# zhoujun-7/VPHO

Measured on AMD Instinct MI355X. Metric: eval images/sec (bs=64, sample_num=100, steps=50); MPJPE delta vs ref, higher is better.
Workload: dtype f32; 1 GPU; vpho_net.forward(mode=predict), README eval config (BASELINE.json configs[1]); per_gpu_batch=64, sample_num=100, sampling_steps=50, topk_hand=30, topk_obj=10, crop=256x256, pipeline_depth=3, parallelism=dp1, score_mfma=f32, conv_mfma=f32, winograd_3x3=True

## Files before the change

### vpho_amd/csrc/conv_igemm.hip

```cpp
#include "common.h"
#include "../../include/vpho_hip.h"
#include <cstdlib>
#include <algorithm>

VPHO_STAMP_DECL(conv)

namespace {

#ifndef CONV_ABLATE
#define CONV_ABLATE 0
#endif
constexpr int BK = 32;
constexpr int LDS_LD = BK + 4;
constexpr int GLDS_PRE_MAX = 512;

struct Geo {
    vpho_conv_desc d;
    int M, K, tiles_m, tiles_n, ntiles;
    int w_ld;
    long long x_zs, w_zs, y_zs;
    long long b_zs, r_zs, x2_zs, pre_zs, ru_zs;
    int y_linear, r_linear, vec_epilogue;
    int uni;
    int dbg;
// ... 540 lines not shown
#pragma unroll
                for (int i = 0; i < TM; ++i)
#pragma unroll
                    for (int j = 0; j < TN; ++j)
                        acc[i][j] = __builtin_amdgcn_mfma_f32_32x32x2f32(a[i][q], b[j][q], acc[i][j], 0, 0, 0);
        }
    };
    VPHO_STAMP_AT(2);
    VPHO_PRIO_MAIN();
    for (int kt = 0; kt + 1 < nk; ++kt) {
        if ((kt > 0 || (g.dbg & 16)) && !(CONV_ABLATE & 64)) { if (UNI) fill_uni((kt & 1) ^ 1, kt + 1); else fill((kt & 1) ^ 1); }
        compute(kt);
        if (!(CONV_ABLATE & 128)) VPHO_SYNC_LDS_DMA();
    }
    if (res_early) { if (d.res_up) load_res_up(); else load_res(); __builtin_amdgcn_sched_barrier(0); }
    compute(nk - 1);
    VPHO_SYNC_LDS_DMA();
    VPHO_PRIO_REST();
    VPHO_STAMP_AT(3);
    if ((CONV_ABLATE & 256) && acc[0][0][0] != 1.2345e-30f) return;

    if (g.vec_epilogue) {
        constexpr int C_LD = BN;
        float* Cs = smem;
        static_assert(BM * C_LD <= 2 * TILE, "epilogue tile does not fit the staging LDS");
#pragma unroll
        for (int j = 0; j < TN; ++j)
#pragma unroll
            for (int i = 0; i < TM; ++i)
#pragma unroll
                for (int e = 0; e < 16; ++e) {
                    const int r = wm * (BM / WM) + i * 32 + (e & 3) + 8 * (e >> 2) + 4 * lh;
                    Cs[r * C_LD + wn * (BN / WN) + j * 32 + li] = acc[i][j][e];
                }
        __syncthreads();
        if (!res_early) { if (d.res_up) load_res_up(); else load_res(); }
        static_assert(NT % V_PER_ROW == 0 && NT >= 2 * BN, "stats layout");
        f32x4 st0 = {0.f, 0.f, 0.f, 0.f}, st1 = {0.f, 0.f, 0.f, 0.f}, piv = st0;
        float cnt = 0.f;
        f32x4 bn_m = st0, bn_i = st0, bn_g = st0, bn_b = st0;
        if (d.bn_x) {
            const int c = n0 + 4 * (tid % V_PER_ROW);
            if (c < d.Cout) {
                bn_m = *reinterpret_cast<const f32x4*>(d.bn_mean + c); bn_i = *reinterpret_cast<const f32x4*>(d.bn_invstd + c);
                if (!d.gate) { bn_g = *reinterpret_cast<const f32x4*>(d.bn_gamma + c); bn_b = *reinterpret_cast<const f32x4*>(d.bn_beta + c); }
            }
        }
#pragma unroll
        for (int it = 0; it < ITERS; ++it) {
            long long yoff, ro;
            if (!item(it, yoff, ro)) continue;
            const int idx = tid + it * NT;
            const int r = idx / V_PER_ROW, c4 = idx - r * V_PER_ROW;
            const f32x4 v = *reinterpret_cast<const f32x4*>(Cs + r * C_LD + 4 * c4);
            f32x4 bv = {0.f, 0.f, 0.f, 0.f};
            if (d.bias) bv = *reinterpret_cast<const f32x4*>(d.bias + n0 + 4 * c4);
            f32x4 o;
#pragma unroll
            for (int k = 0; k < 4; ++k) { const float t = v[k] + bv[k] + rv[it][k]; o[k] = t > 0.f ? t : t * d.out_slope; }
            if (d.gate) {
                const f32x4 gt = *reinterpret_cast<const f32x4*>(d.gate + yoff);
#pragma unroll
                for (int k = 0; k < 4; ++k) o[k] = gt[k] > 0.f ? o[k] : o[k] * d.gate_slope;
            }
            if (d.bn_x) {
                const f32x4 xv = *reinterpret_cast<const f32x4*>(d.bn_x + yoff);
#pragma unroll
                for (int k = 0; k < 4; ++k) {
                    const float xh = (xv[k] - bn_m[k]) * bn_i[k];
                    if (!d.gate) {
                        const float t = xh * bn_g[k] + bn_b[k];
                        o[k] = t > 0.f ? o[k] : o[k] * d.gate_slope;
                    }
                    st0[k] += o[k]; st1[k] += o[k] * xh;
                }
            } else if (d.stats) {
                if (it == 0) {
#pragma unroll
                    for (int k = 0; k < 4; ++k) piv[k] = __shfl(o[k], lane & (V_PER_ROW - 1));
                }
                cnt += 1.f;
#pragma unroll
                for (int k = 0; k < 4; ++k) { const float dv = o[k] - piv[k]; st0[k] += dv; st1[k] += dv * dv; }
            }
            *reinterpret_cast<f32x4*>(d.y + yoff) = o;
        }
        if (d.stats) {
            static_assert(V_PER_ROW == 16 || V_PER_ROW == 32, "lane layout of the epilogue items");
            constexpr int NWAVES = NT / 64;
            static_assert(4 * NWAVES * BN <= BM * C_LD, "stats staging");
#pragma unroll
            for (int k = 0; k < 4; ++k) {
                if (V_PER_ROW == 16) { st0[k] = sum_lane_bit_4(st0[k]); st1[k] = sum_lane_bit_4(st1[k]); }
                st0[k] = sum_lane_bit_5(st0[k]); st1[k] = sum_lane_bit_5(st1[k]);
            }
            if (!d.bn_x) {
                if (V_PER_ROW == 16) cnt = sum_lane_bit_4(cnt);
                cnt = sum_lane_bit_5(cnt);
            }
            __syncthreads();
            float* R = smem;
            if (lane < V_PER_ROW) {
                *reinterpret_cast<f32x4*>(R + (wave * 4 + 0) * BN + 4 * lane) = st0;
                *reinterpret_cast<f32x4*>(R + (wave * 4 + 1) * BN + 4 * lane) = st1;
                *reinterpret_cast<f32x4*>(R + (wave * 4 + 2) * BN + 4 * lane) = piv;
                *reinterpret_cast<f32x4*>(R + (wave * 4 + 3) * BN + 4 * lane) = f32x4{cnt, cnt, cnt, cnt};
            }
            __syncthreads();
            if (d.bn_x) {
                if (tid < 2 * BN) {
                    const int pl = tid / BN, c = tid - pl * BN;
                    float t = R[pl * BN + c];
#pragma unroll
                    for (int k = 1; k < NWAVES; ++k) t += R[(k * 4 + pl) * BN + c];
                    if (n0 + c < d.Cout) d.stats[((long long)tile_m * BN_STAT_PLANES + pl) * d.Cout + n0 + c] = t;
                }
            } else if (tid < BN) {
                const int c = tid;
                ShiftSums t{R[2 * BN + c], R[c], R[BN + c], R[3 * BN + c]};
#pragma unroll
                for (int k = 1; k < NWAVES; ++k) t = shift_sums_add(t, ShiftSums{R[(k * 4 + 2) * BN + c], R[(k * 4) * BN + c], R[(k * 4 + 1) * BN + c], R[(k * 4 + 3) * BN + c]});
                if (n0 + c < d.Cout) store_bn_row(d.stats + (long long)tile_m * BN_STAT_PLANES * d.Cout + n0 + c, d.Cout, t);
            }
        }
        VPHO_STAMP_AT(4);
        VPHO_STAMP_WRITE(conv, blockIdx.x);
        return;
    }
    const int row_base = m0 + wm * (BM / WM) + 4 * lh, col_base = n0 + wn * (BN / WN) + li;
#pragma unroll
    for (int j = 0; j < TN; ++j) {
        const int col = col_base + j * 32;
        if (col >= d.Cout) continue;
        const float bv = d.bias ? d.bias[col] : 0.f;
#pragma unroll
        for (int i = 0; i < TM; ++i) {
#pragma unroll
            for (int e = 0; e < 16; ++e) {
                const int row = row_base + i * 32 + (e & 3) + 8 * (e >> 2);
                if (row >= M_live) continue;
                long long yoff, ro;
                offsets(row, yoff, ro);
                float v = acc[i][j][e] + bv;
                if (d.res) v += d.res[ro + col];
                v = v > 0.f ? v : v * d.out_slope;
                if (d.gate) v = d.gate[yoff + col] > 0.f ? v : v * d.gate_slope;
                d.y[yoff + col] = v;
            }
        }
    }
}

#define VPHO_WAIT_VM(n) asm volatile("s_waitcnt vmcnt(%0)" :: "n"(n) : "memory")
template <int BM, int BN, int WM, int WN, bool STATS>
__device__ __forceinline__ void conv_pers_body(const Geo& g) {
    constexpr int NT = 64 * WM * WN, NW = WM * WN;
    constexpr int TM = BM / (32 * WM), TN = BN / (32 * WN);
    constexpr int ROWS = NT / 8;
    constexpr int A_LD = BM / ROWS, B_LD = BN / ROWS, NF = A_LD + B_LD;
    static_assert(TM >= 1 && TN >= 1 && A_LD >= 1 && B_LD >= 1 && ROWS % 16 == 0 && BN / WN <= 64, "tile/wave layout");
    constexpr int TILE = (BM + BN) * BK;
    constexpr int EPI = 8 * 32;
    constexpr int NIT = TM * 4 * TN;
    __shared__ __attribute__((aligned(1024))) float smem[2 * TILE + NW * EPI + 2 * BN];
    VPHO_STAMP_INIT();

    vpho_conv_desc d = g.d;
    advance_group(d, g, blockIdx.y);
    const int tid = threadIdx.x, lane = tid & 63, wave = __builtin_amdgcn_readfirstlane(tid >> 6);
    const int li = lane & 31, lh = lane >> 5;
    const int wm = wave / WN, wn = wave % WN;
    const int lrow = wave * 8 + (lane >> 3);
    const int kq = (lane & 7) ^ ((lrow >> 1) & 7);
    const int ohw = d.OH * d.OW;
    const __amdgpu_buffer_rsrc_t xu = __builtin_amdgcn_make_buffer_rsrc(const_cast<float*>(d.x), 0, 0xFFFFFFF0u, 0x00020000);
    const __amdgpu_buffer_rsrc_t wr = __builtin_amdgcn_make_buffer_rsrc(const_cast<float*>(d.w), 0, 0xFFFFFFF0u, 0x00020000);
    const __amdgpu_buffer_rsrc_t x2r = __builtin_amdgcn_make_buffer_rsrc(const_cast<float*>(d.x2 ? d.x2 : d.x), 0, 0xFFFFFFF0u, 0x00020000);
    const __amdgpu_buffer_rsrc_t yr = __builtin_amdgcn_make_buffer_rsrc(d.y, 0, 0xFFFFFFF0u, 0x00020000);
    const __amdgpu_buffer_rsrc_t rr = __builtin_amdgcn_make_buffer_rsrc(const_cast<float*>(d.res ? d.res : d.y), 0, 0xFFFFFFF0u, 0x00020000);
    const __amdgpu_buffer_rsrc_t br = __builtin_amdgcn_make_buffer_rsrc(const_cast<float*>(d.bias ? d.bias : d.w), 0, 0xFFFFFFF0u, 0x00020000);
    typedef __attribute__((address_space(3))) void* lds_ptr;

    const int xcd = blockIdx.x & 7, nslot = gridDim.x >> 3, per_xcd = (g.ntiles + 7) >> 3;
    int lt = blockIdx.x >> 3;
    auto tile_at = [&](int t, int& m0, int& n0) -> bool {
        const int lb = xcd * per_xcd + t;
        if (t >= per_xcd || lb >= g.ntiles) return false;
        const int tile_m = lb / g.tiles_n, tile_n = lb - tile_m * g.tiles_n;
        m0 = tile_m * BM; n0 = tile_n * BN;
        return true;
    };
    int m0, n0;
    if (!tile_at(lt, m0, n0)) return;

    int u_voff[A_LD], u_boff[B_LD], u_voff2[A_LD], bias_off;
    auto setup = [&](int m0_, int n0_) {
#pragma unroll
        for (int j = 0; j < A_LD; ++j) {
            const int m = m0_ + lrow + ROWS * j;
            u_voff[j] = -1; u_voff2[j] = -1;
            if (m < g.M) {
                const int n = m / ohw, rem = m - n * ohw;
                const int oy = rem / d.OW, ox = rem - oy * d.OW;
                u_voff[j] = (int)((((long long)(n * d.H + oy * d.stride) * d.W + ox * d.stride) * d.x_ld) * 4 + 16 * kq);
                if (d.x2) u_voff2[j] = (int)((((long long)(n * d.H2 + oy * d.stride2) * d.W2 + ox * d.stride2) * d.x2_ld) * 4 + 16 * kq);
            }
        }
#pragma unroll
        for (int j = 0; j < B_LD; ++j) {
            const int n = n0_ + lrow + ROWS * j;
            u_boff[j] = n < d.Cout ? (int)(((long long)n * g.w_ld + 4 * kq) * 4) : -1;
        }
        const int bc = n0_ + wn * (BN / WN) + lane;
        bias_off = (d.bias && lane < BN / WN && bc < d.Cout) ? bc * 4 : -1;
    };
    auto fill = [&](int buf, int kt, int tp) {
        float* As = smem + buf * TILE + wave * 8 * BK;
        float* Bs = smem + buf * TILE + BM * BK + wave * 8 * BK;
        if (d.x2 && kt * BK >= d.Cin) {
            const int c2 = (kt * BK - d.Cin) * 4;
#pragma unroll
            for (int j = 0; j < A_LD; ++j) {
                const int vo = u_voff2[j];
                __builtin_amdgcn_raw_ptr_buffer_load_lds(x2r, (lds_ptr)(As + ROWS * j * BK), 16, vo, c2, 0, 0);
            }
        } else {
            const int c1 = kt * BK * 4;
#pragma unroll
            for (int j = 0; j < A_LD; ++j) {
                const int vo = u_voff[j];
                __builtin_amdgcn_raw_ptr_buffer_load_lds(xu, (lds_ptr)(As + ROWS * j * BK), 16, vo, c1, 0, 0);
            }
        }
        const int koff = kt * BK * 4;
#pragma unroll
        for (int j = 0; j < B_LD; ++j) {
            const int bo = u_boff[j];
            __builtin_amdgcn_raw_ptr_buffer_load_lds(wr, (lds_ptr)(Bs + ROWS * j * BK), 16, bo, koff, 0, 0);
        }
        if (kt == 0) {
            const int bo = bias_off;
            __builtin_amdgcn_raw_ptr_buffer_load_lds(br, (lds_ptr)(smem + 2 * TILE + NW * EPI + tp * BN + wn * (BN / WN)), 4, bo, 0, 0, 0);
        }
    };

    const int nk = (g.K + BK - 1) / BK;
    const int sw = (li >> 1) & 7;
    f32x16 acc[TM][TN];
    auto compute = [&](int kt) {
        const int buf = kt & 1;
        const float* As = smem + buf * TILE + (wm * (BM / WM) + li) * BK;
        const float* Bs = smem + buf * TILE + BM * BK + (wn * (BN / WN) + li) * BK;
#pragma unroll
        for (int kk = 0; kk < BK / 8; ++kk) {
            const int ch = ((2 * kk + lh) ^ sw) * 4;
            f32x4 a[TM], b[TN];
#pragma unroll
            for (int i = 0; i < TM; ++i) a[i] = *reinterpret_cast<const f32x4*>(As + i * 32 * BK + ch);
#pragma unroll
            for (int j = 0; j < TN; ++j) b[j] = *reinterpret_cast<const f32x4*>(Bs + j * 32 * BK + ch);
#pragma unroll
            for (int q = 0; q < 4; ++q)
#pragma unroll
                for (int i = 0; i < TM; ++i)
#pragma unroll
                    for (int j = 0; j < TN; ++j)
                        acc[i][j] = __builtin_amdgcn_mfma_f32_32x32x2f32(a[i][q], b[j][q], acc[i][j], 0, 0, 0);
        }
    };

    float* Cw = smem + 2 * TILE + wave * EPI;
    const int er = lane >> 3, ec = (lane & 7) * 4;
    auto item_off = [&](int m0_, int n0_, int i, int gq, int j, int& yo, int& ro) {
        const int row = m0_ + wm * (BM / WM) + i * 32 + 8 * gq + er, col = n0_ + wn * (BN / WN) + j * 32 + ec;
        yo = ro = -1;
        if (row < g.M && col < d.Cout) {
            long long y_, r_;
            if (g.y_linear && g.r_linear) { y_ = (long long)row * d.y_sx; r_ = (long long)row * d.r_sx; }
            else {
                const int n = row / ohw, rem = row - n * ohw;
                const int oy = rem / d.OW, ox = rem - oy * d.OW;
                y_ = n * d.y_sn + oy * d.y_sy + ox * d.y_sx; r_ = n * d.r_sn + oy * d.r_sy + ox * d.r_sx;
            }
            yo = (int)((y_ + col) * 4);
            if (d.res) ro = (int)((r_ + col) * 4);
        }
    };

    constexpr bool stats_on = STATS;
    static_assert(4 * (BN / WN) <= EPI && BN <= NT, "stats layout");
    auto flush_stats = [&](int m0_, int n0_) {
        if (tid < BN) {
            const int c = tid;
            const int wn_c = c / (BN / WN), cc = c - wn_c * (BN / WN);
            const float* q = smem + 2 * TILE + wn_c * EPI + cc;
            constexpr int PL = BN / WN;
            ShiftSums t{q[2 * PL], q[0], q[PL], q[3 * PL]};
#pragma unroll
            for (int w = 1; w < WM; ++w) {
                const float* r = q + w * WN * EPI;
                t = shift_sums_add(t, ShiftSums{r[2 * PL], r[0], r[PL], r[3 * PL]});
            }
            if (n0_ + c < d.Cout) store_bn_row(d.stats + (long long)(m0_ / BM) * BN_STAT_PLANES * d.Cout + n0_ + c, d.Cout, t);
        }
    };
    int pm0 = 0, pn0 = 0;

    int tp = 0;
    setup(m0, n0);
    fill(0, 0, tp);
    if (nk > 1) fill(1, 1, tp);
    VPHO_STAMP_AT(1);
    bool first = true;
    while (true) {
        if (nk > 1) { if (first) VPHO_WAIT_VM(NF); else VPHO_WAIT_VM(NF + NIT); }
        else        { if (first) VPHO_WAIT_VM(0);  else VPHO_WAIT_VM(NIT); }
        VPHO_BARRIER_LDS_ONLY();
        if (stats_on && !first) flush_stats(pm0, pn0);
        if (first) VPHO_STAMP_AT(2);
        VPHO_PRIO_MAIN();
#pragma unroll
        for (int i = 0; i < TM; ++i)
#pragma unroll
            for (int j = 0; j < TN; ++j)
#pragma unroll
                for (int e = 0; e < 16; ++e) acc[i][j][e] = 0.f;
        for (int kt = 0; kt + 1 < nk; ++kt) {
            if (kt > 0) fill((kt & 1) ^ 1, kt + 1, tp);
            compute(kt);
            VPHO_SYNC_LDS_DMA();
        }
        f32x4 rv[NIT];
#pragma unroll
        for (int i = 0; i < TM; ++i)
#pragma unroll
            for (int gq = 0; gq < 4; ++gq)
#pragma unroll
                for (int j = 0; j < TN; ++j) {
                    int yo, ro;
                    item_off(m0, n0, i, gq, j, yo, ro);
                    rv[(i * 4 + gq) * TN + j] = __builtin_bit_cast(f32x4, __builtin_amdgcn_raw_buffer_load_b128(rr, ro, 0, 0));
                }
        __builtin_amdgcn_sched_barrier(0);
        compute(nk - 1);
        VPHO_SYNC_LDS_DMA();
#pragma unroll
        for (int k = 0; k < NIT; ++k) asm volatile("" :: "v"(rv[k]));
        VPHO_PRIO_REST();
        if (first) VPHO_STAMP_AT(3);
        const int em0 = m0, en0 = n0, etp = tp;
        lt += nslot;
        const bool more = tile_at(lt, m0, n0);
        if (more) {
            tp ^= 1;
            setup(m0, n0);
            fill(0, 0, tp);
            if (nk > 1) fill(1, 1, tp);
        }
        const float* Bq = smem + 2 * TILE + NW * EPI + etp * BN + wn * (BN / WN) + ec;
        f32x4 st0[TN], st1[TN], piv[TN];
#pragma unroll
        for (int j = 0; j < TN; ++j) { st0[j] = f32x4{0.f, 0.f, 0.f, 0.f}; st1[j] = st0[j]; piv[j] = st0[j]; }
#pragma unroll
        for (int i = 0; i < TM; ++i)
#pragma unroll
            for (int gq = 0; gq < 4; ++gq)
#pragma unroll
                for (int j = 0; j < TN; ++j) {
#pragma unroll
                    for (int e4 = 0; e4 < 4; ++e4) Cw[(e4 + 4 * lh) * 32 + li] = acc[i][j][4 * gq + e4];
                    int yo, ro;
                    item_off(em0, en0, i, gq, j, yo, ro);
                    const f32x4 v = *reinterpret_cast<const f32x4*>(Cw + er * 32 + ec);
                    const f32x4 bq = *reinterpret_cast<const f32x4*>(Bq + j * 32);
                    const f32x4 r = rv[(i * 4 + gq) * TN + j];
                    f32x4 o;
#pragma unroll
                    for (int k = 0; k < 4; ++k) { const float t = v[k] + bq[k] + r[k]; o[k] = t > 0.f ? t : t * d.out_slope; }
                    __builtin_amdgcn_raw_buffer_store_b128(__builtin_bit_cast(__attribute__((__vector_size__(4 * sizeof(unsigned)))) unsigned, o), yr, yo, 0, 0);
                    if (stats_on) {
                        if (i == 0 && gq == 0) {
#pragma unroll
                            for (int k = 0; k < 4; ++k) piv[j][k] = __shfl(o[k], lane & 7);
                        }
#pragma unroll
                        for (int k = 0; k < 4; ++k) { const float u = yo != -1 ? o[k] - piv[j][k] : 0.f; st0[j][k] += u; st1[j][k] += u * u; }
                    }
                }
        if (stats_on) {
            const float n = (float)max(0, min(BM / WM, g.M - (em0 + wm * (BM / WM))));
            static_assert(TM * 32 == BM / WM, "a wave's rows are one block");
#pragma unroll
            for (int j = 0; j < TN; ++j) {
#pragma unroll
                for (int k = 0; k < 4; ++k) { st0[j][k] = sum_lane_bits_345(st0[j][k]); st1[j][k] = sum_lane_bits_345(st1[j][k]); }
                if (lane < 8) {
                    *reinterpret_cast<f32x4*>(Cw + j * 32 + ec) = st0[j];
                    *reinterpret_cast<f32x4*>(Cw + (BN / WN) + j * 32 + ec) = st1[j];
                    *reinterpret_cast<f32x4*>(Cw + 2 * (BN / WN) + j * 32 + ec) = piv[j];
                    *reinterpret_cast<f32x4*>(Cw + 3 * (BN / WN) + j * 32 + ec) = f32x4{n, n, n, n};
                }
            }
            pm0 = em0; pn0 = en0;
        }
        if (first) { VPHO_STAMP_AT(4); }
        first = false;
        if (!more) break;
    }
    if (stats_on) { VPHO_BARRIER_LDS_ONLY(); flush_stats(pm0, pn0); }
    VPHO_STAMP_WRITE(conv, blockIdx.x);
}
template <int BM, int BN, int WM, int WN>
__global__ __launch_bounds__(64 * WM * WN, 4) void conv_igemm_pers_kernel(const Geo g) { conv_pers_body<BM, BN, WM, WN, false>(g); }
template <int BM, int BN, int WM, int WN>
__global__ __launch_bounds__(64 * WM * WN, 4) void conv_igemm_pers_bn_kernel(const Geo g) { conv_pers_body<BM, BN, WM, WN, true>(g); }

typedef __bf16 cbf16x8 __attribute__((ext_vector_type(8)));
constexpr int SBK = 16;

__device__ __forceinline__ void conv_split3(const f32x4& x0, const f32x4& x1, cbf16x8& h, cbf16x8& m, cbf16x8& l) {
#pragma unroll
    for (int e = 0; e < 8; ++e) {
        const float x = e < 4 ? x0[e] : x1[e - 4];
        const __bf16 hb = (__bf16)x;
        const float r1 = x - (float)hb;
        const __bf16 mb = (__bf16)r1;
        const float r2 = r1 - (float)mb;
        h[e] = hb; m[e] = mb; l[e] = (__bf16)r2;
    }
}

template <int BM, int BN, int WM, int WN, int TERMS>
__global__ __launch_bounds__(64 * WM * WN) void conv_igemm_split_kernel(const Geo g) {
    constexpr int NT = 64 * WM * WN, NW = WM * WN;
    constexpr int TM = BM / (32 * WM), TN = BN / (32 * WN);
    constexpr int A_ROWS = NW * 16;
    constexpr int A_LD = BM / A_ROWS;
    constexpr int B_ROWS = NW * 32;
    constexpr int B_PASSES = (3 * BN + B_ROWS - 1) / B_ROWS;
    static_assert(TM >= 1 && TN >= 1 && A_LD >= 1 && BM % A_ROWS == 0, "tile/wave layout");
    constexpr int A_FLOATS = BM * SBK, PLANE_FLOATS = BN * SBK / 2;
    constexpr int TILE = A_FLOATS + 3 * PLANE_FLOATS;
    constexpr int EPI_FLOATS = BM * BN;
    __shared__ __attribute__((aligned(1024))) float smem[(2 * TILE > EPI_FLOATS) ? 2 * TILE : EPI_FLOATS];

    vpho_conv_desc d = g.d;
    int per_xcd = gridDim.x >> 3, ntiles = g.ntiles, M_live = g.M;
    if (d.row_map) {
        M_live = min(*d.row_count, g.M);
        ntiles = (M_live + BM - 1) / BM * g.tiles_n;
        per_xcd = (ntiles + 7) >> 3;
        if ((int)(blockIdx.x >> 3) >= per_xcd) return;
    }
    const int lb = (blockIdx.x & 7) * per_xcd + (blockIdx.x >> 3);
    if (lb >= ntiles) return;
    const int tile_n = lb % g.tiles_n, tile_m = lb / g.tiles_n;
    const int m0 = tile_m * BM, n0 = tile_n * BN;

    const int tid = threadIdx.x, lane = tid & 63, wave = __builtin_amdgcn_readfirstlane(tid >> 6);
    const int li = lane & 31, lh = lane >> 5;
    const int wm = wave / WN, wn = wave % WN;
    const int ohw = d.OH * d.OW;

    const long long pad_shift = ((long long)d.pad_y * d.W + d.pad_x) * d.x_ld;
    const __amdgpu_buffer_rsrc_t xu = __builtin_amdgcn_make_buffer_rsrc(
        reinterpret_cast<void*>(reinterpret_cast<uintptr_t>(d.x) - (uintptr_t)(pad_shift * 4)), 0, 0xFFFFFFF0u, 0x00020000);
    const int arow = wave * 16 + (lane >> 2);
    int a_iy0[A_LD], a_ix0[A_LD], u_voff[A_LD];
#pragma unroll
    for (int j = 0; j < A_LD; ++j) {
        const int lr = arow + A_ROWS * j;
        int m = m0 + lr;
        const int kq = (lane & 3) ^ ((lr >> 2) & 3);
        if (m < M_live) {
            if (d.row_map) m = d.row_map[m];
            const int n = m / ohw, rem = m - n * ohw;
            const int oy = rem / d.OW, ox = rem - oy * d.OW;
            a_iy0[j] = oy * d.stride - d.pad_y;
            a_ix0[j] = ox * d.stride - d.pad_x;
            const unsigned off = (unsigned)(((long long)(n * d.H + a_iy0[j]) * d.W + a_ix0[j]) * d.x_ld * 4);
            u_voff[j] = (int)(off + (unsigned)(pad_shift * 4) + 16u * (unsigned)kq);
        } else {
            a_iy0[j] = -(1 << 28); a_ix0[j] = 0; u_voff[j] = -1;
        }
    }
    const __amdgpu_buffer_rsrc_t wr = __builtin_amdgcn_make_buffer_rsrc(const_cast<void*>(d.w_planes), 0, 0xFFFFFFF0u, 0x00020000);
    int b_voff[B_PASSES];
#pragma unroll
    for (int ps = 0; ps < B_PASSES; ++ps) {
        const int fr = wave * 32 + (lane >> 1) + B_ROWS * ps;
        const int plane = fr / BN, r = fr - plane * BN, n = n0 + r;
        const int ch = (lane & 1) ^ ((r >> 3) & 1);
        b_voff[ps] = (plane < 3 && n < d.Cout) ? (int)((((long long)plane * d.Cout + n) * g.w_ld + ch * 8) * 2) : -1;
    }
    const bool simple = d.KH == 1 && d.KW == 1 && d.pad_y == 0 && d.pad_x == 0;
    int u_r = 0, u_s = 0, u_c = 0;
    typedef __attribute__((address_space(3))) void* lds_ptr;
    auto fill = [&](int buf, int kt) {
        float* As = smem + buf * TILE + wave * 16 * SBK;
        float* Bs = smem + buf * TILE + A_FLOATS + wave * 32 * (SBK / 2);
        const int tap_s = ((u_r * d.W + u_s) * d.x_ld + u_c) * 4;
#pragma unroll
        for (int j = 0; j < A_LD; ++j) {
            int off = u_voff[j];
            if (!simple) {
                const unsigned iy = (unsigned)(a_iy0[j] + u_r), ix = (unsigned)(a_ix0[j] + u_s);
                off = (iy < (unsigned)d.H && ix < (unsigned)d.W) ? off : -1;
            }
            __builtin_amdgcn_raw_ptr_buffer_load_lds(xu, (lds_ptr)(As + A_ROWS * j * SBK), 16, off, tap_s, 0, 0);
        }
        const int koff = kt * SBK * 2;
#pragma unroll
        for (int ps = 0; ps < B_PASSES; ++ps) {
            if (wave * 32 + B_ROWS * ps < 3 * BN) {
                const int bo = b_voff[ps];
                __builtin_amdgcn_raw_ptr_buffer_load_lds(wr, (lds_ptr)(Bs + B_ROWS * ps * (SBK / 2)), 16, bo, koff, 0, 0);
            }
        }
        u_c += SBK;
        if (u_c >= d.Cin) { u_c = 0; if (++u_s == d.KW) { u_s = 0; ++u_r; } }
    };

    f32x16 acc[TM][TN];
#pragma unroll
    for (int i = 0; i < TM; ++i)
#pragma unroll
        for (int j = 0; j < TN; ++j)
#pragma unroll
            for (int e = 0; e < 16; ++e) acc[i][j][e] = 0.f;

    struct Frag { cbf16x8 ah[TM], am[TM], al[TM]; cbf16x8 b[TN][3]; };
    const int a_sw = (li >> 2) & 3, b_sw = (li >> 3) & 1;
    auto read_frags = [&](int buf, Frag& f) {
        const float* As = smem + buf * TILE + (wm * (BM / WM) + li) * SBK;
        const __bf16* Bp = reinterpret_cast<const __bf16*>(smem + buf * TILE + A_FLOATS) + (wn * (BN / WN) + li) * SBK + ((lh ^ b_sw) * 8);
#pragma unroll
        for (int j = 0; j < TN; ++j)
#pragma unroll
            for (int p = 0; p < 3; ++p) f.b[j][p] = *reinterpret_cast<const cbf16x8*>(Bp + (p * BN + j * 32) * SBK);
#pragma unroll
        for (int i = 0; i < TM; ++i) {
            const f32x4 x0 = *reinterpret_cast<const f32x4*>(As + i * 32 * SBK + ((2 * lh) ^ a_sw) * 4);
            const f32x4 x1 = *reinterpret_cast<const f32x4*>(As + i * 32 * SBK + ((2 * lh + 1) ^ a_sw) * 4);
            conv_split3(x0, x1, f.ah[i], f.am[i], f.al[i]);
        }
    };
    auto products = [&](const Frag& f) {
#pragma unroll
        for (int i = 0; i < TM; ++i)
#pragma unroll
            for (int j = 0; j < TN; ++j) {
                if (TERMS == 9) {
                    acc[i][j] = __builtin_amdgcn_mfma_f32_32x32x16_bf16(f.al[i], f.b[j][2], acc[i][j], 0, 0, 0);
                    acc[i][j] = __builtin_amdgcn_mfma_f32_32x32x16_bf16(f.am[i], f.b[j][2], acc[i][j], 0, 0, 0);
                    acc[i][j] = __builtin_amdgcn_mfma_f32_32x32x16_bf16(f.al[i], f.b[j][1], acc[i][j], 0, 0, 0);
                }
                acc[i][j] = __builtin_amdgcn_mfma_f32_32x32x16_bf16(f.al[i], f.b[j][0], acc[i][j], 0, 0, 0);
                acc[i][j] = __builtin_amdgcn_mfma_f32_32x32x16_bf16(f.ah[i], f.b[j][2], acc[i][j], 0, 0, 0);
                acc[i][j] = __builtin_amdgcn_mfma_f32_32x32x16_bf16(f.am[i], f.b[j][1], acc[i][j], 0, 0, 0);
                acc[i][j] = __builtin_amdgcn_mfma_f32_32x32x16_bf16(f.am[i], f.b[j][0], acc[i][j], 0, 0, 0);
                acc[i][j] = __builtin_amdgcn_mfma_f32_32x32x16_bf16(f.ah[i], f.b[j][1], acc[i][j], 0, 0, 0);
                acc[i][j] = __builtin_amdgcn_mfma_f32_32x32x16_bf16(f.ah[i], f.b[j][0], acc[i][j], 0, 0, 0);
            }
    };

    const int nk = g.K / SBK;
    Frag fr[2];
    fill(0, 0);
// ... 68 lines not shown
        *reinterpret_cast<f32x4*>(d.y + yo[it]) = o;
    }
}

}

extern "C" int vpho_conv2d_nhwc_f32(const vpho_conv_desc* dp, void* stream) {
    VPHO_REQUIRE(dp != nullptr, "vpho_conv2d_nhwc_f32: null descriptor");
    const vpho_conv_desc& d = *dp;
    VPHO_REQUIRE(d.x && d.w && d.y, "vpho_conv2d_nhwc_f32: null tensor");
    VPHO_REQUIRE(d.N > 0 && d.H > 0 && d.W > 0 && d.Cin > 0 && d.Cout > 0 && d.KH > 0 && d.KW > 0 && d.stride > 0,
                 "vpho_conv2d_nhwc_f32: non-positive dimension");
    VPHO_REQUIRE(d.Cin % 4 == 0 && d.x_ld % 4 == 0 && d.x_ld >= d.Cin, "vpho_conv2d_nhwc_f32: Cin=%d x_ld=%d must be multiples of 4, x_ld>=Cin", d.Cin, d.x_ld);
    VPHO_REQUIRE(((uintptr_t)d.x & 15) == 0 && ((uintptr_t)d.w & 15) == 0, "vpho_conv2d_nhwc_f32: x/w must be 16-byte aligned");
    VPHO_REQUIRE((d.in_scale == nullptr) == (d.in_shift == nullptr), "vpho_conv2d_nhwc_f32: in_scale/in_shift must come together");
    VPHO_REQUIRE(d.in_scale == nullptr || (((uintptr_t)d.in_scale & 15) == 0 && ((uintptr_t)d.in_shift & 15) == 0), "vpho_conv2d_nhwc_f32: in_scale/in_shift alignment");
    VPHO_REQUIRE(d.OH > 0 && d.OW > 0, "vpho_conv2d_nhwc_f32: empty output");
    VPHO_REQUIRE((d.OH - 1) * d.stride - d.pad_y < d.H && (d.OW - 1) * d.stride - d.pad_x < d.W, "vpho_conv2d_nhwc_f32: output larger than input allows");
    long long M = (long long)d.N * d.OH * d.OW;
    VPHO_REQUIRE(M < (1ll << 31), "vpho_conv2d_nhwc_f32: too many output pixels");
    Geo g;
    g.d = d;
    g.M = (int)M;
    g.K = d.KH * d.KW * d.Cin + (d.x2 ? d.Cin2 : 0);
    const int splits = d.splits > 1 ? d.splits : 1;
    g.w_ld = d.w_ld > 0 ? d.w_ld : g.K;
    g.x_zs = splits > 1 ? d.x_split : 0; g.w_zs = splits > 1 ? d.w_split : 0; g.y_zs = splits > 1 ? d.y_split : 0;
    g.b_zs = g.r_zs = g.x2_zs = g.pre_zs = g.ru_zs = 0;
    const int groups = d.groups > 1 ? d.groups : 1;
    if (groups > 1) {
        VPHO_REQUIRE(splits == 1 && !d.row_map && !d.gate && !d.w_planes, "vpho_conv2d_nhwc_f32: grouped launches take no splits / pixel list / gate / bf16 planes");
        VPHO_REQUIRE(d.x_group >= 0 && d.w_group > 0 && d.y_group > 0 && d.x_group % 4 == 0 && d.w_group % 4 == 0 && d.y_group % 4 == 0 && d.bias_group % 4 == 0 &&
                     d.res_group % 4 == 0 && d.x2_group % 4 == 0 && d.pre_group % 4 == 0 && d.ru_group % 4 == 0,
                     "vpho_conv2d_nhwc_f32: group strides must be non-negative multiples of 4 floats (x_group may be 0: a shared input)");
        g.x_zs = d.x_group; g.w_zs = d.w_group; g.y_zs = d.y_group; g.b_zs = d.bias_group; g.r_zs = d.res_group; g.x2_zs = d.x2_group;
        g.pre_zs = d.pre_group; g.ru_zs = d.ru_group;
    }
    const int ny = splits * groups;
    VPHO_REQUIRE(g.w_ld >= g.K && g.w_ld % 4 == 0 && g.x_zs % 4 == 0 && g.w_zs % 4 == 0, "vpho_conv2d_nhwc_f32: w_ld / split strides must be multiples of 4, w_ld >= K");
    VPHO_REQUIRE(splits == 1 || (!d.res && !d.bias && !d.in_scale && !d.gate), "vpho_conv2d_nhwc_f32: split launches produce plain partial sums (no bias / residual / prologue / gate)");
    g.y_linear = (d.y_sy == d.y_sx * d.OW && d.y_sn == d.y_sy * d.OH) ? 1 : 0;
    g.r_linear = (d.res == nullptr) || (d.r_sy == d.r_sx * d.OW && d.r_sn == d.r_sy * d.OH) ? 1 : 0;
    VPHO_REQUIRE((d.row_map == nullptr) == (d.row_count == nullptr), "vpho_conv2d_nhwc_f32: row_map / row_count must come together");
    if (d.row_map) {
        VPHO_REQUIRE(splits == 1 && !d.gate, "vpho_conv2d_nhwc_f32: pixel-list launches take no splits / gate");
        if (!d.rows_scatter) g.y_linear = g.r_linear = 1;
    }
    auto al16 = [](const void* p) { return ((uintptr_t)p & 15) == 0; };
    g.vec_epilogue = (d.Cout % 4 == 0 && al16(d.y) && d.y_sx % 4 == 0 && d.y_sy % 4 == 0 && d.y_sn % 4 == 0 &&
                      (!d.bias || al16(d.bias)) &&
                      (!d.gate || al16(d.gate)) &&
                      (!d.res || (al16(d.res) && d.r_sx % 4 == 0 && d.r_sy % 4 == 0 && d.r_sn % 4 == 0))) ? 1 : 0;
    const char* dbg_env = getenv("VPHO_CONV_DBG");
    g.dbg = dbg_env ? (atoi(dbg_env) & (8 | 16)) : 0;
    if (d.x2) {
        VPHO_REQUIRE(d.KH == 1 && d.KW == 1 && d.pad_y == 0 && d.pad_x == 0 && d.Cin % BK == 0 && d.Cin2 > 0 && d.Cin2 % BK == 0 && d.x2_ld % 4 == 0 &&
                     d.x2_ld >= d.Cin2 && d.stride2 > 0 && al16(d.x2) && !d.row_map && !d.in_scale && splits == 1 && !d.w_planes,
                     "vpho_conv2d_nhwc_f32: x2 needs a 1x1 unpadded convolution, Cin and Cin2 multiples of 32, no pixel list / prologue / splits / planes");
        VPHO_REQUIRE((d.OH - 1) * d.stride2 < d.H2 && (d.OW - 1) * d.stride2 < d.W2 && 4.0 * d.N * d.H2 * d.W2 * (double)d.x2_ld < 3.9e9,
                     "vpho_conv2d_nhwc_f32: x2 of %d x %d pixels read at stride %d does not cover the %d x %d output (or exceeds 3.9 GB)", d.H2, d.W2, d.stride2, d.OH, d.OW);
    }
    if (d.res_up) {
        VPHO_REQUIRE(!d.res && !d.gate && splits == 1 && d.ru_H > 0 && d.ru_W > 0 && d.ru_ld >= d.Cout && d.ru_ld % 4 == 0 && al16(d.res_up),
                     "vpho_conv2d_nhwc_f32: res_up needs no res / gate / splits, a (N, ru_H, ru_W, ru_ld >= Cout) map with ru_ld %% 4 == 0, 16-byte aligned");
        VPHO_REQUIRE(g.vec_epilogue && d.in_scale == nullptr && !d.w_planes && (!d.row_map || d.rows_scatter),
                     "vpho_conv2d_nhwc_f32: res_up needs 16-byte addressable output rows, no prologue affine, no split-bf16 planes, scattered pixel lists");
        VPHO_REQUIRE(4.0 * d.N * d.ru_H * d.ru_W * (double)d.ru_ld < 3.9e9, "vpho_conv2d_nhwc_f32: res_up map too large");
    }
    hipStream_t s = (hipStream_t)stream;
    if (d.stats_rows) *d.stats_rows = 0;
    const bool stats_shape = g.vec_epilogue && splits == 1 && groups == 1 && !d.row_map && !d.w_planes && (d.in_scale == nullptr);
    if (d.bn_x) {
        VPHO_REQUIRE(d.stats && d.stats_rows && d.bn_mean && d.bn_invstd && (d.gate || (d.bn_gamma && d.bn_beta)),
                     "vpho_conv2d_nhwc_f32: bn_x needs stats, stats_rows, mean / invstd and -- without a stored gate -- gamma / beta");
        VPHO_REQUIRE((stats_shape || d.gate) && al16(d.bn_x) && al16(d.bn_mean) && al16(d.bn_invstd) && (!d.bn_gamma || (al16(d.bn_gamma) && al16(d.bn_beta))),
                     "vpho_conv2d_nhwc_f32: bn_x without a stored gate is served by the direct-to-LDS 16-byte epilogue only (Cout %% 4 == 0, aligned, no splits / groups / pixel list / prologue / planes)");
    }
    VPHO_REQUIRE(!d.stats || (d.stats_rows && d.stats_cap > 0 && al16(d.stats)), "vpho_conv2d_nhwc_f32: stats needs stats_rows (host) and stats_cap");
    const long long big_tiles = ((M + 127) / 128) * ((d.Cout + 127) / 128) * ny;
    const double m_acc = (d.row_map && d.rows_hint > 0) ? (double)d.rows_hint : (double)M;
    const double flops = 2.0 * m_acc * d.Cout * g.K * ny;
    const double bytes = groups * 4.0 * ((double)d.N * d.H * d.W * d.Cin + (d.x2 ? (double)d.N * d.OH * d.OW * d.Cin2 : 0.0) + (double)d.Cout * g.K + m_acc * d.Cout * (d.res ? 2 : 1) + d.Cout + (d.res_up ? (double)d.N * d.ru_H * d.ru_W * d.Cout : 0.0));
    static const int force_tile = getenv("VPHO_CONV_TILE") ? atoi(getenv("VPHO_CONV_TILE")) : 0;
    const long long tiles_12864 = ((M + 127) / 128) * ((d.Cout + 63) / 64) * ny;
    int variant = 64;
    if (big_tiles >= 256 && d.Cout % 128 == 0) variant = 1288;
    else if (tiles_12864 >= 256 && d.Cout >= 48) variant = 12864;
    if (force_tile) variant = force_tile;
    bool stats_kernel = false, stats_failed = false;
    auto launch = [&](auto kernel, int bm, int bn, int threads, int cls) {
        vpho::ProfScope prof(cls, s, flops, bytes);
        g.tiles_m = (int)((M + bm - 1) / bm); g.tiles_n = (d.Cout + bn - 1) / bn;
        g.ntiles = g.tiles_m * g.tiles_n;
        if (d.stats) {
            const bool on = stats_kernel && stats_shape && g.tiles_m <= d.stats_cap;
            if (on) {
                *d.stats_rows = g.tiles_m;
                if (d.bn_x && d.bn_gamma) g.d.gate = nullptr;
            } else {
                g.d.stats = nullptr;
                if (d.bn_x) { if (!d.gate) { stats_failed = true; return; } g.d.bn_x = nullptr; }
            }
        }
        hipLaunchKernelGGL(kernel, dim3((g.ntiles + 7) / 8 * 8, ny), dim3(threads), 0, s, g);
    };
    static const int no_glds = getenv("VPHO_CONV_NO_GLDS") ? atoi(getenv("VPHO_CONV_NO_GLDS")) : 0;
    const double x_extent = 4.0 * (((double)d.N * d.H * d.W - 1) * d.x_ld + d.Cin + (double)(ny - 1) * (double)g.x_zs);
    const double w_extent = 4.0 * (((double)d.Cout - 1) * g.w_ld + g.K + (double)(ny - 1) * (double)g.w_zs);
    VPHO_REQUIRE(x_extent < 3.9e9 && w_extent < 3.9e9 && g.x_zs >= 0 && g.w_zs >= 0,
                 "vpho_conv2d_nhwc_f32: input (%.2f GB) and weights (%.2f GB) must each stay below 3.9 GB", x_extent * 1e-9, w_extent * 1e-9);
    static const int no_uni = getenv("VPHO_CONV_NO_UNI") ? atoi(getenv("VPHO_CONV_NO_UNI")) : 0;
    g.uni = (d.Cin % BK == 0 && d.pad_y >= 0 && d.pad_x >= 0 && !no_uni) ? 1 : 0;
    const bool pre_on_read = d.in_scale != nullptr && g.uni && d.KH == 1 && d.KW == 1 && d.pad_y == 0 && d.pad_x == 0 && d.Cin <= GLDS_PRE_MAX;
    const bool glds = (d.in_scale == nullptr || pre_on_read) && (!no_glds || d.res_up != nullptr || d.x2 != nullptr || d.bn_x != nullptr);
    stats_kernel = glds && variant != 128;
    VPHO_REQUIRE(!d.x2 || (g.uni && variant != 128), "vpho_conv2d_nhwc_f32: x2 is served by the direct-to-LDS kernels with wave-uniform taps only");
    VPHO_REQUIRE(!d.res_up || variant != 128, "vpho_conv2d_nhwc_f32: res_up is not served by the forced register-staged tile");
    const bool split_ok = d.w_planes != nullptr && (d.plane_terms == 6 || d.plane_terms == 9) && d.in_scale == nullptr && splits == 1 && !d.gate &&
                          d.Cin % SBK == 0 && g.vec_epilogue && d.pad_y >= 0 && d.pad_x >= 0 && g.w_ld == g.K &&
                          ((uintptr_t)d.w_planes & 15) == 0 && 6.0 * d.Cout * g.K < 3.9e9;
    if (split_ok) {
        const bool x9 = d.plane_terms == 9;
        switch (variant) {
            case 128: case 1288:
                if (x9) launch(conv_igemm_split_kernel<128, 128, 4, 2, 9>, 128, 128, 512, vpho::PROF_CONV128);
                else    launch(conv_igemm_split_kernel<128, 128, 4, 2, 6>, 128, 128, 512, vpho::PROF_CONV128);
                break;
            case 12864:
                if (x9) launch(conv_igemm_split_kernel<128, 64, 4, 2, 9>, 128, 64, 512, vpho::PROF_CONV128x64);
                else    launch(conv_igemm_split_kernel<128, 64, 4, 2, 6>, 128, 64, 512, vpho::PROF_CONV128x64);
                break;
            default:
                if (x9) launch(conv_igemm_split_kernel<64, 64, 2, 2, 9>, 64, 64, 256, vpho::PROF_CONV64);
                else    launch(conv_igemm_split_kernel<64, 64, 2, 2, 6>, 64, 64, 256, vpho::PROF_CONV64);
                break;
        }
        return vpho::check_launch("conv_igemm_split_kernel");
    }
    {
        const char* pe = getenv("VPHO_CONV_PERS");
        const int pers = pe ? atoi(pe) : 1;
        static int slots_of[64] = {0};
        int dev = 0;
        VPHO_HIP(hipGetDevice(&dev));
        int& slots = slots_of[dev & 63];
        if (!slots) {
            hipDeviceProp_t prop;
            VPHO_HIP(hipGetDeviceProperties(&prop, dev));
            slots = 2 * prop.multiProcessorCount;
        }
        const double y_extent = 4.0 * ((double)(d.N - 1) * d.y_sn + (double)(d.OH - 1) * d.y_sy + (double)(d.OW - 1) * d.y_sx + d.Cout);
        const double r_extent = d.res ? 4.0 * ((double)(d.N - 1) * d.r_sn + (double)(d.OH - 1) * d.r_sy + (double)(d.OW - 1) * d.r_sx + d.Cout) : 0.0;
        const bool simple = d.KH == 1 && d.KW == 1 && d.pad_y == 0 && d.pad_x == 0;
        const bool ok = pers && variant == 1288 && glds && !pre_on_read && d.in_scale == nullptr && g.uni && simple && g.vec_epilogue && !d.row_map && !d.res_up &&
                        !d.gate && !d.bn_x && splits == 1 && y_extent < 3.9e9 && r_extent < 3.9e9 && d.y_sn >= 0 && d.y_sy >= 0 && d.y_sx >= 0 &&
                        (!d.x2 || 4.0 * d.N * d.H2 * d.W2 * (double)d.x2_ld < 3.9e9);
        if (ok && (big_tiles > slots || pers >= 2)) {
            vpho::ProfScope prof(vpho::PROF_CONV128, s, flops, bytes);
            g.tiles_m = (int)((M + 127) / 128); g.tiles_n = (d.Cout + 127) / 128;
            g.ntiles = g.tiles_m * g.tiles_n;
            if (d.stats) {
                if (stats_shape && g.tiles_m <= d.stats_cap) *d.stats_rows = g.tiles_m; else g.d.stats = nullptr;
            }
            const int grid = (int)std::min<long long>((g.ntiles + 7) / 8 * 8, std::max(8, slots / groups / 8 * 8));
            if (g.d.stats) hipLaunchKernelGGL((conv_igemm_pers_bn_kernel<128, 128, 4, 2>), dim3(grid, groups), dim3(512), 0, s, g);
            else hipLaunchKernelGGL((conv_igemm_pers_kernel<128, 128, 4, 2>), dim3(grid, groups), dim3(512), 0, s, g);
            return vpho::check_launch("conv_igemm_pers_kernel");
        }
    }
    switch (variant) {
        case 128:  launch(conv_igemm_kernel<128, 128, 2, 2, 1>, 128, 128, 256, vpho::PROF_CONV128); break;
        case 1288:
            if (glds && pre_on_read) launch(conv_igemm_glds_kernel<128, 128, 4, 2, true>, 128, 128, 512, vpho::PROF_CONV128);
            else if (glds) launch(conv_igemm_glds_kernel<128, 128, 4, 2>, 128, 128, 512, vpho::PROF_CONV128);
            else      launch(conv_igemm_kernel<128, 128, 4, 2, 1>, 128, 128, 512, vpho::PROF_CONV128);
            break;
        case 12864:
            if (glds && pre_on_read) launch(conv_igemm_glds_kernel<128, 64, 4, 2, true>, 128, 64, 512, vpho::PROF_CONV128x64);
            else if (glds) launch(conv_igemm_glds_kernel<128, 64, 4, 2>, 128, 64, 512, vpho::PROF_CONV128x64);
            else      launch(conv_igemm_kernel<128, 64, 4, 2, 1>, 128, 64, 512, vpho::PROF_CONV128x64);
            break;
        default:
            if (glds && pre_on_read) launch(conv_igemm_glds_kernel<64, 64, 2, 2, true>, 64, 64, 256, vpho::PROF_CONV64);
            else if (glds) launch(conv_igemm_glds_kernel<64, 64, 2, 2>, 64, 64, 256, vpho::PROF_CONV64);
            else      launch(conv_igemm_kernel<64, 64, 2, 2, 1>, 64, 64, 256, vpho::PROF_CONV64);
            break;
    }
    if (stats_failed)
        return vpho::fail("vpho_conv2d_nhwc_f32: bn_x: the launch needs %d partial rows (stats_cap %d) or runs a kernel without the BatchNorm epilogue (tile %d)",
                          g.tiles_m, d.stats_cap, variant);
    return vpho::check_launch("conv_igemm_kernel");
}
```

Measured before the change: 2228 images/s.

## Add persistent conv variants for fused bilinear upsample-add and A-tile reuse

Adds two variants of the persistent 1x1 conv kernel. The LAT variant fuses a bilinear-upsampled residual add, with optional row-map scatter, into the epilogue, so those convs no longer fall back to the non-persistent path. The RESA variant walks all N tiles of one M row-block on a block and skips reloading the A operand when K is small. This adds template complexity and register pressure, and the RESA waitcnt accounting is a correctness risk.

```diff
diff --git a/vpho_amd/csrc/conv_igemm.hip b/vpho_amd/csrc/conv_igemm.hip
--- a/vpho_amd/csrc/conv_igemm.hip
+++ b/vpho_amd/csrc/conv_igemm.hip
@@ -716,7 +716,7 @@
 }
 
 #define VPHO_WAIT_VM(n) asm volatile("s_waitcnt vmcnt(%0)" :: "n"(n) : "memory")
-template <int BM, int BN, int WM, int WN, bool STATS>
+template <int BM, int BN, int WM, int WN, bool STATS, bool RESA = false, bool LAT = false>
 __device__ __forceinline__ void conv_pers_body(const Geo& g) {
     constexpr int NT = 64 * WM * WN, NW = WM * WN;
     constexpr int TM = BM / (32 * WM), TN = BN / (32 * WN);
@@ -731,25 +731,33 @@
 
     vpho_conv_desc d = g.d;
     advance_group(d, g, blockIdx.y);
+    if constexpr (LAT) { d.x2 = nullptr; d.res = nullptr; }
     const int tid = threadIdx.x, lane = tid & 63, wave = __builtin_amdgcn_readfirstlane(tid >> 6);
     const int li = lane & 31, lh = lane >> 5;
     const int wm = wave / WN, wn = wave % WN;
-    const int lrow = wave * 8 + (lane >> 3);
-    const int kq = (lane & 7) ^ ((lrow >> 1) & 7);
+    const int lrow_k = wave * 8 + (lane >> 3);
+    const int kq_k = (lane & 7) ^ ((lrow_k >> 1) & 7);
     const int ohw = d.OH * d.OW;
     const __amdgpu_buffer_rsrc_t xu = __builtin_amdgcn_make_buffer_rsrc(const_cast<float*>(d.x), 0, 0xFFFFFFF0u, 0x00020000);
     const __amdgpu_buffer_rsrc_t wr = __builtin_amdgcn_make_buffer_rsrc(const_cast<float*>(d.w), 0, 0xFFFFFFF0u, 0x00020000);
     const __amdgpu_buffer_rsrc_t x2r = __builtin_amdgcn_make_buffer_rsrc(const_cast<float*>(d.x2 ? d.x2 : d.x), 0, 0xFFFFFFF0u, 0x00020000);
     const __amdgpu_buffer_rsrc_t yr = __builtin_amdgcn_make_buffer_rsrc(d.y, 0, 0xFFFFFFF0u, 0x00020000);
-    const __amdgpu_buffer_rsrc_t rr = __builtin_amdgcn_make_buffer_rsrc(const_cast<float*>(d.res ? d.res : d.y), 0, 0xFFFFFFF0u, 0x00020000);
+    const __amdgpu_buffer_rsrc_t rr = __builtin_amdgcn_make_buffer_rsrc(const_cast<float*>(LAT ? d.res_up : d.res ? d.res : d.y), 0, 0xFFFFFFF0u, 0x00020000);
     const __amdgpu_buffer_rsrc_t br = __builtin_amdgcn_make_buffer_rsrc(const_cast<float*>(d.bias ? d.bias : d.w), 0, 0xFFFFFFF0u, 0x00020000);
     typedef __attribute__((address_space(3))) void* lds_ptr;
 
-    const int xcd = blockIdx.x & 7, nslot = gridDim.x >> 3, per_xcd = (g.ntiles + 7) >> 3;
+    int M_live = g.M, ntiles = g.ntiles;
+    if (LAT && d.row_map) { M_live = min(*d.row_count, g.M); ntiles = (M_live + BM - 1) / BM * g.tiles_n; }
+    const int xcd = blockIdx.x & 7, nslot = gridDim.x >> 3, per_xcd = ((RESA ? g.tiles_m : ntiles) + 7) >> 3;
     int lt = blockIdx.x >> 3;
     auto tile_at = [&](int t, int& m0, int& n0) -> bool {
         const int lb = xcd * per_xcd + t;
-        if (t >= per_xcd || lb >= g.ntiles) return false;
+        if (RESA) {
+            if (t >= per_xcd || lb >= g.tiles_m) return false;
+            m0 = lb * BM; n0 = 0;
+            return true;
+        }
+        if (t >= per_xcd || lb >= ntiles) return false;
         const int tile_m = lb / g.tiles_n, tile_n = lb - tile_m * g.tiles_n;
         m0 = tile_m * BM; n0 = tile_n * BN;
         return true;
@@ -758,18 +766,27 @@
     if (!tile_at(lt, m0, n0)) return;
 
     int u_voff[A_LD], u_boff[B_LD], u_voff2[A_LD], bias_off;
-    auto setup = [&](int m0_, int n0_) {
+    auto setup = [&](int m0_, int n0_, bool rows) {
+        int lrow = lrow_k, kq = kq_k;
+        if constexpr (LAT) {
+            int l = lane;
+            asm volatile("" : "+v"(l));
+            lrow = wave * 8 + (l >> 3); kq = (l & 7) ^ ((lrow >> 1) & 7);
+        }
+        if (rows) {
 #pragma unroll
         for (int j = 0; j < A_LD; ++j) {
-            const int m = m0_ + lrow + ROWS * j;
+            int m = m0_ + lrow + ROWS * j;
             u_voff[j] = -1; u_voff2[j] = -1;
-            if (m < g.M) {
+            if (m < M_live) {
+                if (LAT && d.row_map) m = d.row_map[m];
                 const int n = m / ohw, rem = m - n * ohw;
                 const int oy = rem / d.OW, ox = rem - oy * d.OW;
                 u_voff[j] = (int)((((long long)(n * d.H + oy * d.stride) * d.W + ox * d.stride) * d.x_ld) * 4 + 16 * kq);
                 if (d.x2) u_voff2[j] = (int)((((long long)(n * d.H2 + oy * d.stride2) * d.W2 + ox * d.stride2) * d.x2_ld) * 4 + 16 * kq);
             }
         }
+        }
 #pragma unroll
         for (int j = 0; j < B_LD; ++j) {
             const int n = n0_ + lrow + ROWS * j;
@@ -778,10 +795,21 @@
         const int bc = n0_ + wn * (BN / WN) + lane;
         bias_off = (d.bias && lane < BN / WN && bc < d.Cout) ? bc * 4 : -1;
     };
-    auto fill = [&](int buf, int kt, int tp) {
+    auto fill = [&](int buf, int kt, int tp, bool rows) {
         float* As = smem + buf * TILE + wave * 8 * BK;
         float* Bs = smem + buf * TILE + BM * BK + wave * 8 * BK;
-        if (d.x2 && kt * BK >= d.Cin) {
+        if (!rows) {
+        } else if (RESA) {
+            const bool second = d.x2 && kt * BK >= d.Cin;
+            const __amdgpu_buffer_rsrc_t ar = second ? x2r : xu;
+            const int c = second ? (kt * BK - d.Cin) * 4 : kt * BK * 4;
+#pragma unroll
+            for (int j = 0; j < A_LD; ++j) {
+                const int v1 = u_voff[j], v2 = u_voff2[j];
+                const int vo = second ? v2 : v1;
+                __builtin_amdgcn_raw_ptr_buffer_load_lds(ar, (lds_ptr)(As + ROWS * j * BK), 16, vo, c, 0, 0);
+            }
+        } else if (d.x2 && kt * BK >= d.Cin) {
             const int c2 = (kt * BK - d.Cin) * 4;
 #pragma unroll
             for (int j = 0; j < A_LD; ++j) {
@@ -815,9 +843,11 @@
         const int buf = kt & 1;
         const float* As = smem + buf * TILE + (wm * (BM / WM) + li) * BK;
         const float* Bs = smem + buf * TILE + BM * BK + (wn * (BN / WN) + li) * BK;
+        int sw_ = sw;
+        if constexpr (LAT) asm volatile("" : "+v"(sw_));
 #pragma unroll
         for (int kk = 0; kk < BK / 8; ++kk) {
-            const int ch = ((2 * kk + lh) ^ sw) * 4;
+            const int ch = ((2 * kk + lh) ^ sw_) * 4;
             f32x4 a[TM], b[TN];
 #pragma unroll
             for (int i = 0; i < TM; ++i) a[i] = *reinterpret_cast<const f32x4*>(As + i * 32 * BK + ch);
@@ -834,9 +864,9 @@
     };
 
     float* Cw = smem + 2 * TILE + wave * EPI;
-    const int er = lane >> 3, ec = (lane & 7) * 4;
+    const int er_k = lane >> 3, ec_k = (lane & 7) * 4;
     auto item_off = [&](int m0_, int n0_, int i, int gq, int j, int& yo, int& ro) {
-        const int row = m0_ + wm * (BM / WM) + i * 32 + 8 * gq + er, col = n0_ + wn * (BN / WN) + j * 32 + ec;
+        const int row = m0_ + wm * (BM / WM) + i * 32 + 8 * gq + er_k, col = n0_ + wn * (BN / WN) + j * 32 + ec_k;
         yo = ro = -1;
         if (row < g.M && col < d.Cout) {
             long long y_, r_;
@@ -871,13 +901,14 @@
     int pm0 = 0, pn0 = 0;
 
     int tp = 0;
-    setup(m0, n0);
-    fill(0, 0, tp);
-    if (nk > 1) fill(1, 1, tp);
+    setup(m0, n0, true);
+    fill(0, 0, tp, true);
+    if (nk > 1) fill(1, 1, tp, true);
     VPHO_STAMP_AT(1);
     bool first = true;
+    bool rows = true;
     while (true) {
-        if (nk > 1) { if (first) VPHO_WAIT_VM(NF); else VPHO_WAIT_VM(NF + NIT); }
+        if (nk > 1) { if (first) VPHO_WAIT_VM(NF); else if (RESA && !rows) VPHO_WAIT_VM(B_LD + NIT); else VPHO_WAIT_VM(NF + NIT); }
         else        { if (first) VPHO_WAIT_VM(0);  else VPHO_WAIT_VM(NIT); }
         VPHO_BARRIER_LDS_ONLY();
         if (stats_on && !first) flush_stats(pm0, pn0);
@@ -890,11 +921,49 @@
 #pragma unroll
                 for (int e = 0; e < 16; ++e) acc[i][j][e] = 0.f;
         for (int kt = 0; kt + 1 < nk; ++kt) {
-            if (kt > 0) fill((kt & 1) ^ 1, kt + 1, tp);
+            if (kt > 0) fill((kt & 1) ^ 1, kt + 1, tp, true);
             compute(kt);
             VPHO_SYNC_LDS_DMA();
         }
         f32x4 rv[NIT];
+        int pk[LAT ? TM * 4 : 1];
+        if constexpr (LAT) {
+            const float sy = (float)d.ru_H / (float)d.OH, sx = (float)d.ru_W / (float)d.OW;
+            int l_ = lane;
+            asm volatile("" : "+v"(l_));
+            const int er_ = l_ >> 3, ec_ = (l_ & 7) * 4;
+#pragma unroll
+            for (int i = 0; i < TM; ++i)
+#pragma unroll
+                for (int gq = 0; gq < 4; ++gq) {
+                    int row = m0 + wm * (BM / WM) + i * 32 + 8 * gq + er_;
+                    const bool live = row < M_live;
+                    if (live && d.row_map) row = d.row_map[row];
+                    const int n = row / ohw, rem = row - n * ohw;
+                    const int oy = rem / d.OW, ox = rem - oy * d.OW;
+                    int y0, y1, x0, x1; float ly, lx;
+                    lin_src(oy, sy, d.ru_H, y0, y1, ly);
+                    lin_src(ox, sx, d.ru_W, x0, x1, lx);
+                    const float hy = 1.f - ly, hx = 1.f - lx;
+                    pk[i * 4 + gq] = live ? row : -1;
+#pragma unroll
+                    for (int j = 0; j < TN; ++j) {
+                        const int col = n0 + wn * (BN / WN) + j * 32 + ec_, k = (i * 4 + gq) * TN + j;
+                        rv[k] = f32x4{0.f, 0.f, 0.f, 0.f};
+                        if (live && col < d.Cout) {
+                            const unsigned r0 = (unsigned)(n * d.ru_H + y0) * (unsigned)d.ru_W, r1 = (unsigned)(n * d.ru_H + y1) * (unsigned)d.ru_W;
+                            const unsigned ld4 = (unsigned)d.ru_ld * 4u, c4 = (unsigned)col * 4u;
+                            const f32x4 a00 = __builtin_bit_cast(f32x4, __builtin_amdgcn_raw_buffer_load_b128(rr, (int)((r0 + x0) * ld4 + c4), 0, 0));
+                            const f32x4 a01 = __builtin_bit_cast(f32x4, __builtin_amdgcn_raw_buffer_load_b128(rr, (int)((r0 + x1) * ld4 + c4), 0, 0));
+                            const f32x4 a10 = __builtin_bit_cast(f32x4, __builtin_amdgcn_raw_buffer_load_b128(rr, (int)((r1 + x0) * ld4 + c4), 0, 0));
+                            const f32x4 a11 = __builtin_bit_cast(f32x4, __builtin_amdgcn_raw_buffer_load_b128(rr, (int)((r1 + x1) * ld4 + c4), 0, 0));
+#pragma unroll
+                            for (int u = 0; u < 4; ++u) rv[k][u] = hy * (hx * a00[u] + lx * a01[u]) + ly * (hx * a10[u] + lx * a11[u]);
+                        }
+                        __builtin_amdgcn_sched_barrier(0);
+                    }
+                }
+        } else {
 #pragma unroll
         for (int i = 0; i < TM; ++i)
 #pragma unroll
@@ -905,6 +974,7 @@
                     item_off(m0, n0, i, gq, j, yo, ro);
                     rv[(i * 4 + gq) * TN + j] = __builtin_bit_cast(f32x4, __builtin_amdgcn_raw_buffer_load_b128(rr, ro, 0, 0));
                 }
+        }
         __builtin_amdgcn_sched_barrier(0);
         compute(nk - 1);
         VPHO_SYNC_LDS_DMA();
@@ -913,13 +983,24 @@
         VPHO_PRIO_REST();
         if (first) VPHO_STAMP_AT(3);
         const int em0 = m0, en0 = n0, etp = tp;
-        lt += nslot;
-        const bool more = tile_at(lt, m0, n0);
+        int epk[LAT ? TM * 4 : 1];
+        if constexpr (LAT) {
+#pragma unroll
+            for (int k = 0; k < TM * 4; ++k) epk[k] = pk[k];
+        }
+        bool more;
+        if (RESA && n0 + BN < d.Cout) { n0 += BN; rows = false; more = true; }
+        else { lt += nslot; rows = true; more = tile_at(lt, m0, n0); }
         if (more) {
             tp ^= 1;
-            setup(m0, n0);
-            fill(0, 0, tp);
-            if (nk > 1) fill(1, 1, tp);
+            if (!RESA || rows) { setup(m0, n0, true); fill(0, 0, tp, true); if (nk > 1) fill(1, 1, tp, true); }
+            else { setup(m0, n0, false); fill(0, 0, tp, false); if (nk > 1) fill(1, 1, tp, false); }
+        }
+        int er = er_k, ec = ec_k;
+        if constexpr (LAT) {
+            int l = lane;
+            asm volatile("" : "+v"(l));
+            er = l >> 3; ec = (l & 7) * 4;
         }
         const float* Bq = smem + 2 * TILE + NW * EPI + etp * BN + wn * (BN / WN) + ec;
         f32x4 st0[TN], st1[TN], piv[TN];
@@ -934,7 +1015,20 @@
 #pragma unroll
                     for (int e4 = 0; e4 < 4; ++e4) Cw[(e4 + 4 * lh) * 32 + li] = acc[i][j][4 * gq + e4];
                     int yo, ro;
-                    item_off(em0, en0, i, gq, j, yo, ro);
+                    if constexpr (LAT) {
+                        const int row = epk[i * 4 + gq], col = en0 + wn * (BN / WN) + j * 32 + ec;
+                        yo = -1;
+                        if (row >= 0 && col < d.Cout) {
+                            long long y_;
+                            if (g.y_linear) y_ = (long long)row * d.y_sx;
+                            else {
+                                const int n = row / ohw, rem = row - n * ohw;
+                                const int oy = rem / d.OW, ox = rem - oy * d.OW;
+                                y_ = n * d.y_sn + oy * d.y_sy + ox * d.y_sx;
+                            }
+                            yo = (int)((y_ + col) * 4);
+                        }
+                    } else item_off(em0, en0, i, gq, j, yo, ro);
                     const f32x4 v = *reinterpret_cast<const f32x4*>(Cw + er * 32 + ec);
                     const f32x4 bq = *reinterpret_cast<const f32x4*>(Bq + j * 32);
                     const f32x4 r = rv[(i * 4 + gq) * TN + j];
@@ -978,6 +1072,10 @@
 __global__ __launch_bounds__(64 * WM * WN, 4) void conv_igemm_pers_kernel(const Geo g) { conv_pers_body<BM, BN, WM, WN, false>(g); }
 template <int BM, int BN, int WM, int WN>
 __global__ __launch_bounds__(64 * WM * WN, 4) void conv_igemm_pers_bn_kernel(const Geo g) { conv_pers_body<BM, BN, WM, WN, true>(g); }
+template <int BM, int BN, int WM, int WN>
+__global__ __launch_bounds__(64 * WM * WN, 4) void conv_igemm_pers_a_kernel(const Geo g) { conv_pers_body<BM, BN, WM, WN, false, true>(g); }
+template <int BM, int BN, int WM, int WN>
+__global__ __launch_bounds__(64 * WM * WN, 4) void conv_igemm_pers_lat_kernel(const Geo g) { conv_pers_body<BM, BN, WM, WN, false, false, true>(g); }
 
 typedef __bf16 cbf16x8 __attribute__((ext_vector_type(8)));
 constexpr int SBK = 16;
@@ -1352,18 +1450,27 @@
         const double y_extent = 4.0 * ((double)(d.N - 1) * d.y_sn + (double)(d.OH - 1) * d.y_sy + (double)(d.OW - 1) * d.y_sx + d.Cout);
         const double r_extent = d.res ? 4.0 * ((double)(d.N - 1) * d.r_sn + (double)(d.OH - 1) * d.r_sy + (double)(d.OW - 1) * d.r_sx + d.Cout) : 0.0;
         const bool simple = d.KH == 1 && d.KW == 1 && d.pad_y == 0 && d.pad_x == 0;
-        const bool ok = pers && variant == 1288 && glds && !pre_on_read && d.in_scale == nullptr && g.uni && simple && g.vec_epilogue && !d.row_map && !d.res_up &&
+        const bool cls = variant == 1288 || (pers >= 2 && !force_tile && d.Cout % 128 == 0);
+        const char* pl = getenv("VPHO_CONV_PERS_LAT");
+        const bool lat = d.res_up != nullptr && (pl ? atoi(pl) : 1) != 0 && !d.res && !d.x2 && !d.stats && (!d.row_map || d.rows_scatter);
+        const long long live_tiles = (((long long)m_acc + 127) / 128) * ((d.Cout + 127) / 128) * ny;
+        const bool ok = pers && cls && glds && !pre_on_read && d.in_scale == nullptr && g.uni && simple && g.vec_epilogue && ((!d.row_map && !d.res_up) || lat) &&
                         !d.gate && !d.bn_x && splits == 1 && y_extent < 3.9e9 && r_extent < 3.9e9 && d.y_sn >= 0 && d.y_sy >= 0 && d.y_sx >= 0 &&
                         (!d.x2 || 4.0 * d.N * d.H2 * d.W2 * (double)d.x2_ld < 3.9e9);
-        if (ok && (big_tiles > slots || pers >= 2)) {
+        if (ok && ((lat ? live_tiles : big_tiles) > slots || pers >= 2)) {
             vpho::ProfScope prof(vpho::PROF_CONV128, s, flops, bytes);
             g.tiles_m = (int)((M + 127) / 128); g.tiles_n = (d.Cout + 127) / 128;
             g.ntiles = g.tiles_m * g.tiles_n;
             if (d.stats) {
                 if (stats_shape && g.tiles_m <= d.stats_cap) *d.stats_rows = g.tiles_m; else g.d.stats = nullptr;
             }
-            const int grid = (int)std::min<long long>((g.ntiles + 7) / 8 * 8, std::max(8, slots / groups / 8 * 8));
-            if (g.d.stats) hipLaunchKernelGGL((conv_igemm_pers_bn_kernel<128, 128, 4, 2>), dim3(grid, groups), dim3(512), 0, s, g);
+            const char* pa = getenv("VPHO_CONV_PERS_A");
+            const bool res_a = !lat && (pa ? atoi(pa) : 1) != 0 && g.K <= 2 * BK && g.tiles_n >= 2 && !g.d.stats;
+            const int units = res_a ? g.tiles_m : g.ntiles;
+            const int grid = (int)std::min<long long>((units + 7) / 8 * 8, std::max(8, slots / groups / 8 * 8));
+            if (lat) hipLaunchKernelGGL((conv_igemm_pers_lat_kernel<128, 128, 4, 2>), dim3(grid, groups), dim3(512), 0, s, g);
+            else if (res_a) hipLaunchKernelGGL((conv_igemm_pers_a_kernel<128, 128, 4, 2>), dim3(grid, groups), dim3(512), 0, s, g);
+            else if (g.d.stats) hipLaunchKernelGGL((conv_igemm_pers_bn_kernel<128, 128, 4, 2>), dim3(grid, groups), dim3(512), 0, s, g);
             else hipLaunchKernelGGL((conv_igemm_pers_kernel<128, 128, 4, 2>), dim3(grid, groups), dim3(512), 0, s, g);
             return vpho::check_launch("conv_igemm_pers_kernel");
         }
```

After: 2245 images/s (median of 6 runs). About the same (+0.7%).
